# GestaltCogTeam/STEP

Hardware: AMD Instinct MI355X
Metric: training windows/sec on PEMS04, horizon-12 MAE parity, 1/2/4/8 MI355X (higher is better)
Workload: dtype f16 (TSFormer Q/K/weights) + bf16 (P, V, GraphWaveNet / graph-learner GEMMs) operands, f32 accumulate

## Files before the change

include/step_hip.h:

```cpp
#ifndef STEP_HIP_H
#define STEP_HIP_H

#include <stdint.h>

#ifdef __cplusplus
extern "C" {
#endif

const char* step_last_error(void);
int step_abi_version(void);

typedef struct StepGemm {
    int M, N, K, batch;
    const void* A; long sam, sak, sab; int a_bf16;
    const void* B; long sbk, sbn, sbb; int b_bf16;
    float* C; long ldc, scn, scb;
    float alpha;
    int accumulate;
    const float* bias; int relu;
    int splitk;
    int a_kblk; long a_kstride;
    int b_kblk; long b_kstride;
    int b_nblk; long b_nstride;
    int c_nblk; long c_nstride;
// ... 34 lines not shown
    float *fc_w, *fc_b;
    float *bn1_w, *bn1_b, *bn1_rm, *bn1_rv;
    float *bn2_w, *bn2_b, *bn2_rm, *bn2_rv;
    float *bn3_w, *bn3_b, *bn3_rm, *bn3_rv;
    float *fc_out_w, *fc_out_b;
    float *fc_cat_w, *fc_cat_b;
    int gemm_bf16;
} StepDglParams;

long step_dgl_global_saved_floats(int N, int T);
long step_dgl_global_work_floats(int N, int T, int backward);
int step_dgl_global_forward(const float* series_nt, int N, int T, const StepDglParams* p, int training,
                            float momentum, float* saved, float* work, float* g, void* stream);
int step_dgl_global_backward(const float* series_nt, int N, int T, const StepDglParams* p, const float* saved,
                             const float* dg, float* work, const StepDglParams* grads, void* stream);
#define STEP_DGL_FRESH_FC_GRAD 16
int step_dgl_global_backward_phase(const float* series_nt, int N, int T, const StepDglParams* p, const float* saved,
                             const float* dg, float* work, const StepDglParams* grads, int phase, void* stream);

typedef struct StepDglShard { int own1; double count1, count2; } StepDglShard;
int step_dgl_global_forward_shard(const float* series_slice, int N, int Ts, const StepDglParams* p, int training, float momentum,
                                  float* saved, float* work, double* sums, float* g, const StepDglShard* shard, int phase,
                                  void* stream);
int step_dgl_global_backward_shard(const float* series_slice, int N, int Ts, const StepDglParams* p, const float* saved,
                                   const float* dg, float* work, const StepDglParams* grads, const StepDglShard* shard, int phase,
                                   void* stream);
long step_dgl_global_offset(int N, int T, int item);

long step_dgl_edges_saved_floats(int B, int N);
long step_dgl_edges_work_floats(int N);
long step_dgl_edges_theta_offset(int N);
int step_dgl_edges_forward(const float* g, int N, int B, const StepDglParams* p, const float* u, uint64_t seed,
                           float temperature, float* saved, float* theta_out, float* adj_out, void* stream);
int step_dgl_edges_backward(const float* g, int N, int B, const StepDglParams* p, const float* saved,
                            const float* dtheta, const float* dadj, float temperature, float* work,
                            const StepDglParams* grads, float* dg, void* aux_stream, void* stream);

typedef struct StepGwnetParams {
    float *nodevec1, *nodevec2;
    float *start_w, *start_b;
    float *filter_w[8], *filter_b[8];
    float *gate_w[8], *gate_b[8];
    float *skip_w[8], *skip_b[8];
    float *bn_w[8], *bn_b[8], *bn_rm[8], *bn_rv[8];
    float *gconv_w[8], *gconv_b[8];
    float *fc_his0_w, *fc_his0_b, *fc_his2_w, *fc_his2_b;
    float *end1_w, *end1_b, *end2_w, *end2_b;
    int gemm_bf16;
} StepGwnetParams;

long step_gwnet_saved_floats(int B, int N, int dropout);
long step_gwnet_work_floats(int B, int N, int backward);
long step_gwnet_saved_offset(int B, int N, int dropout, int item, int layer);
int step_gwnet_forward(const float* hist, int B, int N, int Cin, const float* hidden_last, const float* adj,
                       const StepGwnetParams* p, int training, float dropout_p, uint64_t seed, float momentum,
                       float* saved, float* work, float* pred, void* stream);
int step_gwnet_forward_phase(const float* hist, int B, int N, int Cin, const float* hidden_last, const float* adj,
                             const StepGwnetParams* p, int training, float dropout_p, uint64_t seed, float momentum,
                             float* saved, float* work, float* pred, int phase, void* stream);
int step_gwnet_backward(const float* hist, int B, int N, int Cin, const float* hidden_last, const StepGwnetParams* p,
                        const float* saved, float* work, const float* dpred, const StepGwnetParams* grads,
                        float* dadj, int dropout, void* aux_stream, void* leaf_stream, void* stream);

int step_pt_dropout(const float* x, float* y, long n, float p, uint64_t seed, uint32_t site, void* stream);
int step_pt_ffn_hidden_fwd(const float* x, const float* w1, const float* b1, long R, float p, uint64_t seed, uint32_t site,
                           uint16_t* hidden, void* stream);
int step_pt_ffn_hidden_bwd(const float* dy, const float* w2, const uint16_t* hidden, long R, float p, uint16_t* dhidden, void* stream);
int step_pt_colsum_bf16(const uint16_t* x, long rows, int cols, float* out, void* stream);
long step_pt_rows_linear_pack_bytes(int nkc, int nog);
int step_pt_rows_linear_pack(const float* w, long swo, long swi, int nkc, int nog, const float* bias, void* pack, void* stream);
int step_pt_rows_linear(const void* x, int x_bf16, long R, const void* pack, int nkc, int nog, void* y, int y_bf16, int accumulate, void* stream);
int step_pt_layer_pack(const float* wi, const float* bi, const float* wo, const float* bo, const float* w1, const float* b1, const float* w2,
                       const float* b2, void* ffn, void* qkv, void* o, void* da, void* dx, void* stream);
long step_pt_proj_wgrad_ws_floats(long R);
int step_pt_proj_wgrad(const float* x, const uint16_t* dqkv, const float* dov, const uint16_t* a, long R, float* ws, float* dwi, float* dbi, float* dwo,
                       void* stream);
int step_pt_ffn_fused_fwd_ln(const float* h1, long R, const void* pack, float p, const uint64_t* pool, long pool_words, uint64_t seed, uint32_t site_hidden,
                             uint32_t site_out, const float* gamma, const float* beta, float* pre, float* y, float* stats, void* stream);
int step_pt_rows_linear_ln(const uint16_t* x, long R, const void* pack, const float* res, float p, uint64_t seed, uint32_t site, const float* gamma,
                           const float* beta, float* pre, float* y, float* stats, void* stream);
int step_pt_embed_unmasked_fwd(const float* series, const int* um, const float* w, const float* b, const float* pos, long S, int L, int Pu, float p,
                               uint64_t seed, uint32_t site, float* x, void* stream);
int step_pt_embed_unmasked_bwd(const float* dx, const float* series, const int* um, long S, int L, int Pu, float p, uint64_t seed, uint32_t site,
                               float* dpos, float* dw, float* db, void* stream);
int step_pt_dec_input_bwd_sums(const float* dout, long S, int P, int Pu, float p, uint64_t seed, uint32_t site, const int* midx, float* dz, float* dpos,
                               float* dmask, void* stream);
long step_pt_ffn_pack_bytes(void);
long step_pt_ffn_wgrad_workgroups(long R);
long step_pt_ffn_wgrad_ws_floats(long R);
int step_pt_ffn_pack(const float* w1, const float* b1, const float* w2, const float* b2, void* pack, void* stream);
int step_pt_ffn_fused_fwd(const float* h1, long R, const void* pack, float p, const uint64_t* pool, long pool_words, uint64_t seed, uint32_t site,
                          float* f2, void* stream);
int step_pt_ffn_fused_bwd_data(const float* df2, const float* h1, long R, const void* pack, float p, const uint64_t* pool, long pool_words,
                               uint64_t seed, uint32_t site, float* dh1, void* stream);
int step_pt_ffn_fused_bwd_weights(const float* df2, const float* h1, long R, const void* pack, const float* b1, float p, const uint64_t* pool,
                                  long pool_words, uint64_t seed, uint32_t site, float* ws, float* dw1, float* db1, float* dw2, void* stream);
int step_pt_dropout_relu_mask(float* d, const float* relu_of, long n, float p, uint64_t seed, uint32_t site, void* stream);
int step_pt_add_dropout(const float* a, const float* b, float* out, long n, float p, uint64_t seed, uint32_t site, void* stream);
int step_pt_add_rows(float* x, long S, int P, const float* vec, const int* idx, void* stream);
int step_pt_sum_over_seq(const float* dx, long S, int ldp, int p_off, int p_cnt, const int* idx, float* dvec, void* stream);
int step_pt_token_gather(const float* src, long S, int P, const int* idx, int T, float scale, float* dst, void* stream);
int step_pt_token_scatter(const float* ddst, long S, int P, const int* idx, int T, float scale, float* dsrc, void* stream);
int step_pt_dec_input(const float* z, const float* mask_token, const float* pos, const int* midx, long S, int P, int Pu,
                      float p, uint64_t seed, uint32_t site, float* out, void* stream);
int step_pt_dec_input_bwd(const float* dout, long S, int P, int Pu, float p, uint64_t seed, uint32_t site, float* dz,
                          float* dm, void* stream);
// ... 97 lines not shown
```

step_amd/_lib.py:

```python
import ctypes
import os

import torch

_HERE = os.path.dirname(os.path.abspath(__file__))
LIB_PATH = os.environ.get("STEP_HIP_LIB") or os.path.join(_HERE, "libstep_hip.so")

_vp, _i, _l, _f, _u64 = ctypes.c_void_p, ctypes.c_int, ctypes.c_long, ctypes.c_float, ctypes.c_uint64


class StepGemm(ctypes.Structure):
    _fields_ = [("M", _i), ("N", _i), ("K", _i), ("batch", _i),
                ("A", _vp), ("sam", _l), ("sak", _l), ("sab", _l), ("a_bf16", _i),
                ("B", _vp), ("sbk", _l), ("sbn", _l), ("sbb", _l), ("b_bf16", _i),
                ("C", _vp), ("ldc", _l), ("scn", _l), ("scb", _l),
                ("alpha", _f), ("accumulate", _i), ("bias", _vp), ("relu", _i), ("splitk", _i),
                ("a_kblk", _i), ("a_kstride", _l), ("b_kblk", _i), ("b_kstride", _l),
                ("b_nblk", _i), ("b_nstride", _l), ("c_nblk", _i), ("c_nstride", _l),
                ("a_kscale", _vp), ("a_kshift", _vp), ("a_kperiod", _i),
                ("batch0", _i), ("sab1", _l), ("sbb1", _l), ("scb1", _l), ("compute_bf16", _i), ("a_rowsum", _vp), ("c_nscale", _vp), ("c_nshift", _vp), ("c_mvec", _vp),
                ("c_nperiod", _i), ("splitk_ws", _vp), ("splitk_ws_floats", _l)]


class StepDglParams(ctypes.Structure):
# ... 7 lines not shown
    _fields_ = [("nodevec1", _vp), ("nodevec2", _vp), ("start_w", _vp), ("start_b", _vp),
                ("filter_w", _vp * 8), ("filter_b", _vp * 8), ("gate_w", _vp * 8), ("gate_b", _vp * 8),
                ("skip_w", _vp * 8), ("skip_b", _vp * 8),
                ("bn_w", _vp * 8), ("bn_b", _vp * 8), ("bn_rm", _vp * 8), ("bn_rv", _vp * 8),
                ("gconv_w", _vp * 8), ("gconv_b", _vp * 8),
                ("fc_his0_w", _vp), ("fc_his0_b", _vp), ("fc_his2_w", _vp), ("fc_his2_b", _vp),
                ("end1_w", _vp), ("end1_b", _vp), ("end2_w", _vp), ("end2_b", _vp), ("gemm_bf16", _i)]


_PD = ctypes.POINTER(StepDglParams)


class StepDynState(ctypes.Structure):
    _fields_ = [("seed_xor", ctypes.c_uint64), ("adam_step", ctypes.c_int32), ("lr", _f), ("gsl_coef", _f), ("reserved", _f)]


class StepDglShard(ctypes.Structure):
    _fields_ = [("own1", ctypes.c_int), ("count1", ctypes.c_double), ("count2", ctypes.c_double)]


_PS = ctypes.POINTER(StepDglShard)
_PG = ctypes.POINTER(StepGwnetParams)

_SIGS = {
    "step_last_error": (ctypes.c_char_p, []),
    "step_abi_version": (_i, []),
    "step_gemm": (_i, [ctypes.POINTER(StepGemm), _vp]),
    "step_tsformer_encode": (_i, [_vp, _i, _i, _vp, _l, _i, _i, _vp, _vp, _vp, _vp, _f, _vp, _l, _u64, _vp, _vp]),
    "step_dropout_pool_fill": (_i, [_vp, _l, _f, _u64, _vp]),
    "step_tsformer_dropout_words": (_l, [_i, _i]),
    "step_gather_windows": (_i, [_vp, _i, _i, _i, _i, _vp, _i, _i, _i, _vp, _vp, _vp, _vp]),
    "step_pack_long_history": (_i, [_vp, _i, _i, _i, _i, _i, _vp, _vp]),
    "step_knn_workspace_bytes": (_l, [_i, _i, _i]),
    "step_knn_graph": (_i, [_vp, _vp, _i, _i, _i, _i, _vp, _vp, _vp, _l, _vp]),
    "step_topk_mask": (_i, [_vp, _i, _i, _i, _vp, _vp, _l, _vp]),
    "step_selftest_mfma": (_i, [_vp, _vp]),
    "step_streams_concurrent": (_i, [_vp, _vp, ctypes.POINTER(_i)]),
    "step_dgl_global_saved_floats": (_l, [_i, _i]),
    "step_dgl_global_work_floats": (_l, [_i, _i, _i]),
    "step_dgl_global_forward": (_i, [_vp, _i, _i, _PD, _i, _f, _vp, _vp, _vp, _vp]),
    "step_dgl_global_backward": (_i, [_vp, _i, _i, _PD, _vp, _vp, _vp, _PD, _vp]),
    "step_dgl_global_backward_phase": (_i, [_vp, _i, _i, _PD, _vp, _vp, _vp, _PD, _i, _vp]),
    "step_dgl_global_forward_shard": (_i, [_vp, _i, _i, _PD, _i, _f, _vp, _vp, _vp, _vp, _PS, _i, _vp]),
    "step_dgl_global_backward_shard": (_i, [_vp, _i, _i, _PD, _vp, _vp, _vp, _PD, _PS, _i, _vp]),
    "step_dgl_global_offset": (_l, [_i, _i, _i]),
    "step_dgl_edges_saved_floats": (_l, [_i, _i]),
    "step_dgl_edges_work_floats": (_l, [_i]),
    "step_dgl_edges_theta_offset": (_l, [_i]),
    "step_dgl_edges_forward": (_i, [_vp, _i, _i, _PD, _vp, _u64, _f, _vp, _vp, _vp, _vp]),
    "step_dgl_edges_backward": (_i, [_vp, _i, _i, _PD, _vp, _vp, _vp, _f, _vp, _PD, _vp, _vp, _vp]),
    "step_gwnet_saved_floats": (_l, [_i, _i, _i]),
    "step_gwnet_work_floats": (_l, [_i, _i, _i]),
    "step_gwnet_saved_offset": (_l, [_i, _i, _i, _i, _i]),
    "step_gwnet_forward": (_i, [_vp, _i, _i, _i, _vp, _vp, _PG, _i, _f, _u64, _f, _vp, _vp, _vp, _vp]),
    "step_gwnet_forward_phase": (_i, [_vp, _i, _i, _i, _vp, _vp, _PG, _i, _f, _u64, _f, _vp, _vp, _vp, _i, _vp]),
    "step_gwnet_backward": (_i, [_vp, _i, _i, _i, _vp, _PG, _vp, _vp, _vp, _PG, _vp, _i, _vp, _vp, _vp]),
    "step_pt_dropout": (_i, [_vp, _vp, _l, _f, _u64, ctypes.c_uint32, _vp]),
    "step_pt_ffn_hidden_fwd": (_i, [_vp, _vp, _vp, _l, _f, _u64, ctypes.c_uint32, _vp, _vp]),
    "step_pt_ffn_hidden_bwd": (_i, [_vp, _vp, _vp, _l, _f, _vp, _vp]),
    "step_pt_colsum_bf16": (_i, [_vp, _l, _i, _vp, _vp]),
    "step_pt_rows_linear_pack_bytes": (_l, [_i, _i]),
    "step_pt_rows_linear_pack": (_i, [_vp, _l, _l, _i, _i, _vp, _vp, _vp]),
    "step_pt_rows_linear": (_i, [_vp, _i, _l, _vp, _i, _i, _vp, _i, _i, _vp]),
    "step_pt_layer_pack": (_i, [_vp] * 14),
    "step_pt_proj_wgrad_ws_floats": (_l, [_l]),
    "step_pt_proj_wgrad": (_i, [_vp, _vp, _vp, _vp, _l, _vp, _vp, _vp, _vp, _vp]),
    "step_pt_ffn_fused_fwd_ln": (_i, [_vp, _l, _vp, _f, _vp, _l, _u64, ctypes.c_uint32, ctypes.c_uint32, _vp, _vp, _vp, _vp, _vp, _vp]),
    "step_pt_rows_linear_ln": (_i, [_vp, _l, _vp, _vp, _f, _u64, ctypes.c_uint32, _vp, _vp, _vp, _vp, _vp, _vp]),
    "step_pt_embed_unmasked_fwd": (_i, [_vp, _vp, _vp, _vp, _vp, _l, _i, _i, _f, _u64, ctypes.c_uint32, _vp, _vp]),
    "step_pt_embed_unmasked_bwd": (_i, [_vp, _vp, _vp, _l, _i, _i, _f, _u64, ctypes.c_uint32, _vp, _vp, _vp, _vp]),
    "step_pt_dec_input_bwd_sums": (_i, [_vp, _l, _i, _i, _f, _u64, ctypes.c_uint32, _vp, _vp, _vp, _vp, _vp]),
    "step_pt_ffn_pack_bytes": (_l, []),
    "step_pt_ffn_wgrad_workgroups": (_l, [_l]),
    "step_pt_ffn_wgrad_ws_floats": (_l, [_l]),
    "step_pt_ffn_pack": (_i, [_vp, _vp, _vp, _vp, _vp, _vp]),
    "step_pt_ffn_fused_fwd": (_i, [_vp, _l, _vp, _f, _vp, _l, _u64, ctypes.c_uint32, _vp, _vp]),
    "step_pt_ffn_fused_bwd_data": (_i, [_vp, _vp, _l, _vp, _f, _vp, _l, _u64, ctypes.c_uint32, _vp, _vp]),
    "step_pt_ffn_fused_bwd_weights": (_i, [_vp, _vp, _l, _vp, _vp, _f, _vp, _l, _u64, ctypes.c_uint32, _vp, _vp, _vp, _vp, _vp]),
    "step_pt_add_layernorm_fwd": (_i, [_vp, _vp, _l, _f, _u64, ctypes.c_uint32, _vp, _vp, _vp, _vp, _vp, _vp]),
    "step_pt_layernorm_bwd_dropout": (_i, [_vp, _vp, _l, _vp, _vp, _vp, _vp, _f, _u64, ctypes.c_uint32, _vp, _vp, _vp, _vp]),
    "step_pt_dropout_relu_mask": (_i, [_vp, _vp, _l, _f, _u64, ctypes.c_uint32, _vp]),
    "step_pt_add_dropout": (_i, [_vp, _vp, _vp, _l, _f, _u64, ctypes.c_uint32, _vp]),
    "step_pt_add_rows": (_i, [_vp, _l, _i, _vp, _vp, _vp]),
    "step_pt_sum_over_seq": (_i, [_vp, _l, _i, _i, _i, _vp, _vp, _vp]),
    "step_pt_token_gather": (_i, [_vp, _l, _i, _vp, _i, _f, _vp, _vp]),
    "step_pt_token_scatter": (_i, [_vp, _l, _i, _vp, _i, _f, _vp, _vp]),
    "step_pt_dec_input": (_i, [_vp, _vp, _vp, _vp, _l, _i, _i, _f, _u64, ctypes.c_uint32, _vp, _vp]),
    "step_pt_dec_input_bwd": (_i, [_vp, _l, _i, _i, _f, _u64, ctypes.c_uint32, _vp, _vp, _vp]),
    "step_pt_layernorm_fwd": (_i, [_vp, _l, _vp, _vp, _vp, _vp, _vp]),
    "step_pt_layernorm_bwd": (_i, [_vp, _vp, _l, _vp, _vp, _vp, _vp, _vp, _vp]),
    "step_pt_attention_fwd": (_i, [_vp, _l, _i, _f, _u64, ctypes.c_uint32, _vp, _vp, _vp]),
    "step_pt_attention_bwd": (_i, [_vp, _vp, _vp, _vp, _l, _i, _f, _u64, ctypes.c_uint32, _vp, _vp]),
    "step_pt_attention_fwd_bf16": (_i, [_vp, _l, _i, _f, _u64, ctypes.c_uint32, _vp, _vp, _vp, _vp, _l, _vp]),
    "step_pt_attention_bwd_bf16": (_i, [_vp, _vp, _vp, _vp, _l, _i, _f, _u64, ctypes.c_uint32, _vp, _vp, _vp]),
    "step_pt_linear_bf16out": (_i, [_vp, _vp, _l, _l, _vp, _l, _i, _i, _vp, _vp]),
    "step_pt_relu_mask": (_i, [_vp, _vp, _l, _vp]),
    "step_colsum": (_i, [_vp, _l, _i, _l, _vp, _vp]),
    "step_loss_fwd_bwd": (_i, [_vp, _vp, _l, _vp, _vp, _l, _f, _f, _vp, _vp, _vp, _vp, _vp]),
    "step_loss_scaled_fwd_bwd": (_i, [_vp, _vp, _l, _l, _f, _f, _vp, _vp, _l, _f, _f, _vp, _vp, _vp, _vp, _vp]),
    "step_scale2": (_i, [_vp, _l, _vp, _l, _vp, _vp, _vp, _vp]),
    "step_masked_metrics": (_i, [_vp, _l, _vp, _l, _l, _f, _vp, _vp, _vp]),
    "step_adam_work_floats": (_l, []),
    "step_adam_clip": (_i, [_vp, _vp, _vp, _vp, _l, _f, _f, _f, _f, _f, _i, _f, _vp, _vp, _vp]),
    "step_adam_clip_sharded": (_i, [_vp, _vp, _vp, _vp, _l, _f, _f, _f, _f, _f, _i, _f, _vp, _vp, _vp, _vp]),
    "step_comm_available": (_i, []),
    "step_comm_version": (_i, []),
# ... 107 lines not shown
```

step_amd/csrc/gwnet.hip:

```cpp
#include "common.h"
#include "step_internal.h"
#include <vector>

namespace {

constexpr int C = 32, CAT = 224, CS = 256, CE = 512, OUT = 12, NL = 8, HID = 96;
constexpr int TIN[NL] = {13, 12, 10, 9, 7, 6, 4, 3};
constexpr int DIL[NL] = {1, 2, 1, 2, 1, 2, 1, 2};
constexpr int TOUT[NL] = {12, 10, 9, 7, 6, 4, 3, 1};

__global__ void start_conv_kernel(const float* __restrict__ hist, int B, int N, int Cin, const float* __restrict__ w,
                                  const float* __restrict__ b, float* __restrict__ x0) {
    long idx = (long)blockIdx.x * 256 + threadIdx.x;
    long total = (long)B * N * 13 * C;
    if (idx >= total) return;
    int c = idx % C, t = (idx / C) % 13;
    long bn = idx / (C * 13);
    int n = bn % N, bb = bn / N;
    float v = b[c];
    if (t >= 1) {
        const float* src = hist + (((long)bb * 12 + (t - 1)) * N + n) * Cin;
        v += w[c * 2] * src[0] + w[c * 2 + 1] * src[1];
    }
    x0[idx] = v;
// ... 529 lines not shown
        for (int e = 0; e < 16; ++e) acc[e] = 0.f;
#pragma unroll
        for (int q = 0; q < 4; ++q) mma16<BF16>(acc, dp[q >> 1][q & 1], b[q]);
#pragma unroll
        for (int e = 0; e < 16; ++e) dxs[(wave & 1) * 32 + (e & 3) + 8 * (e >> 2) + 4 * h][32 * nt + col] = acc[e];
    }
    __syncthreads();
    const int c = threadIdx.x & 31, jg = threadIdx.x >> 5;
    float s1 = 0.f, s2 = 0.f;
    const float mean = statprev ? statprev[64 + c] : 0.f, rstd = statprev ? statprev[96 + c] : 0.f;
    const int njt = G * Tin;
    for (int j0 = 0; j0 < njt; j0 += 32) {
        float dr[4], yv[4], v[4];
        long o[4];
        bool valid[4];
#pragma unroll
        for (int u = 0; u < 4; ++u) {
            const int j = j0 + 8 * u + jg;
            const int g = j / Tin, t = j - g * Tin;
            const long bnr = bn0 + g;
            valid[u] = j < njt && bnr < BN;
            const long bc = valid[u] ? bnr : 0;
            const int tc = valid[u] ? t : 0;
            o[u] = (bc * Tin + tc) * C + c;
            const bool tap1 = valid[u] && tc >= dil;
            dr[u] = (dres && tap1) ? dres[(bc * Tout + tc - dil) * C + c] : 0.f;
            yv[u] = yprev ? yprev[o[u]] : 0.f;
            float x = 0.f;
            if (valid[u] && tc < Tout) x += dxs[g * Tout + tc][c];
            if (tap1) x += dxs[g * Tout + tc - dil][32 + c];
            v[u] = x;
        }
#pragma unroll
        for (int u = 0; u < 4; ++u) {
            if (!valid[u]) continue;
            const float x = v[u] + dr[u];
            dx[o[u]] = x;
            s1 += x; s2 += x * (yv[u] - mean) * rstd;
        }
    }
    if (!yprev) return;
    red[jg][c] = s1; red[jg][32 + c] = s2;
    __syncthreads();
    if (threadIdx.x < 64) {
        float a = 0.f;
#pragma unroll
        for (int r = 0; r < 8; ++r) a += red[r][threadIdx.x];
        bsum[threadIdx.x] = a;
    }
    __syncthreads();
    add_block_sums(sums, bsum);
}

__global__ void im2col_kernel(XIn x, long BN, int Tin, int Tout, int dil, float* __restrict__ xcat) {
    long idx = (long)blockIdx.x * 256 + threadIdx.x;
    if (idx >= BN * Tout * 64) return;
    int k = idx % 64, t = (idx / 64) % Tout;
    long bn = idx / (64L * Tout);
    float v = x.src[(bn * Tin + t + (k >> 5) * dil) * C + (k & 31)];
    if (x.stat) v = v * x.stat[k & 31] + x.stat[32 + (k & 31)];
    xcat[idx] = v;
}
__global__ void unpack_skip_grad_kernel(const float* __restrict__ dwskip, SkipPtrs G) {
    const int o = blockIdx.x, k = threadIdx.x;
    G.w[k >> 5][o * C + (k & 31)] += dwskip[o * CS + k];
}
__global__ void head_combine_kernel(const float* __restrict__ skip, const float* __restrict__ h2, long n, float* __restrict__ xh) {
    long idx = (long)blockIdx.x * 256 + threadIdx.x;
    if (idx >= n) return;
    xh[idx] = fmaxf(skip[idx] + h2[idx], 0.f);
}
struct MPtr8 { float* p[8]; };
__global__ void add_to8_kernel(MPtr8 dst, const float* __restrict__ v, int n) {
    int i = blockIdx.x * 256 + threadIdx.x;
    if (i >= n) return;
    const float x = v[i];
#pragma unroll
    for (int k = 0; k < 8; ++k) dst.p[k][i] += x;
}
__global__ void relu_bwd_kernel(float* __restrict__ d, const float* __restrict__ y, long n) {
    long idx = (long)blockIdx.x * 256 + threadIdx.x;
    if (idx < n && !(y[idx] > 0.f)) d[idx] = 0.f;
}

__global__ __launch_bounds__(256) void rowsum_mod_kernel(const float* __restrict__ x, int cols, int mod, float* __restrict__ out) {
    __shared__ float red[4];
    const long row = blockIdx.x;
    float s = 0.f;
    for (int j = threadIdx.x; j < cols; j += 256) s += x[row * cols + j];
    s = wave_sum(s);
    if ((threadIdx.x & 63) == 0) red[threadIdx.x >> 6] = s;
    __syncthreads();
    if (threadIdx.x == 0) atomicAdd(&out[row % mod], red[0] + red[1] + red[2] + red[3]);
}

constexpr int ADJ_NSEG = 2 * (12 + 10 + 9 + 7 + 6 + 4 + 3);
struct AdjOffsets { long cat[NL - 1], dcat[NL - 1]; };
__global__ void adj_ktab_kernel(AdjOffsets o, int N, GemmKSeg* __restrict__ tab) {
    const int j = threadIdx.x, s = blockIdx.x;
    if (j >= ADJ_NSEG) return;
    constexpr int tout[NL - 1] = {12, 10, 9, 7, 6, 4, 3};
    int i = 0, rem = j >> 1;
    while (rem >= tout[i]) { rem -= tout[i]; ++i; }
    const int t = rem, pair = j & 1, T = tout[i];
    GemmKSeg g;
    g.a_off = o.cat[i] + (long)t * CAT + (pair == 0 ? (1 + 2 * s) * C : 0);
    g.b_off = o.dcat[i] + (long)t * CAT + (pair == 0 ? (2 + 2 * s) * C : (1 + 2 * s) * C);
    g.a_rs = g.b_rs = T * CAT;
    g.a_bs = g.b_bs = (long)N * T * CAT;
    tab[s * ADJ_NSEG + j] = g;
}

inline dim3 g1(long n) { return dim3((unsigned)((n + 255) / 256)); }

// ... 4 lines not shown
    float* take(long n) {
        float* p = base ? base + used : nullptr;
        used += (n + 3) & ~3L;
        return p;
    }
};

static inline int n8(int N) { return (N + 7) & ~7; }
static inline bool hop_transposed_operand(int N) {
    static const int min_n = []() { const char* e = getenv("STEP_HOP_XT_MIN_N"); return e ? atoi(e) : 768; }();
    return N >= min_n;
}

struct Saved {
    float *x0, *cat[NL], *tf[NL], *sg[NL], *y[NL], *mask[NL], *bnstat[NL], *zlast;
    float *Pstk, *PTstk, *Pa, *Madp, *rs, *cs;
    uint16_t *P16, *PT16;
    float *skip, *h1, *h2, *xh, *e1;
    long total;
};
Saved carve_saved(float* base, int B, int N, bool dropout) {
    Carver cv(base);
    Saved s;
    const long BN = (long)B * N;
    s.x0 = cv.take(BN * TIN[0] * C);
    s.zlast = cv.take(BN * CS);
    for (int i = 0; i < NL; ++i) {
        s.cat[i] = cv.take(BN * TOUT[i] * CAT);
        s.tf[i] = cv.take(BN * TOUT[i] * C);
        s.sg[i] = cv.take(BN * TOUT[i] * C);
        s.y[i] = i < NL - 1 ? cv.take(BN * TOUT[i] * C) : nullptr;
        s.mask[i] = (i < NL - 1 && dropout) ? cv.take(BN * TOUT[i] * C) : nullptr;
        s.bnstat[i] = cv.take(128);
    }
    s.Pstk = cv.take(3L * B * N * N);
    s.PTstk = cv.take(3L * B * N * N);
    s.P16 = (uint16_t*)cv.take(3L * B * N * n8(N) / 2);
    s.PT16 = (uint16_t*)cv.take(3L * B * N * n8(N) / 2);
    s.Pa = cv.take((long)N * N);
    s.Madp = cv.take((long)N * N);
    s.rs = cv.take(BN);
    s.cs = cv.take(BN);
    s.skip = cv.take(BN * CS);
    s.h1 = cv.take(BN * CE);
    s.h2 = cv.take(BN * CS);
    s.xh = cv.take(BN * CS);
    s.e1 = cv.take(BN * CE);
    s.total = cv.used;
    return s;
}
struct Work {
    float *wcat, *wcatT, *bcat, *wskip, *wmixT, *dwcat, *dbcat, *dwskip;
    double* acc64;
    float *xcat[NL], *bsum, *y7, *m7;
    uint16_t* xT;
    float *dcat[NL - 1], *dpre[NL], *dh[NL - 1], *dres, *dxa, *dxb, *dskip, *dPstk, *dPa, *dM, *rf, *rb;
    GemmKSeg* ktab;
    float *d_e1, *d_xh, *d_h2, *d_h1;
    long total;
};
Work carve_work(float* base, int B, int N, bool backward) {
    Carver cv(base);
    Work w;
    const long BN = (long)B * N;
    w.wcat = cv.take(NL * 64 * 64);
    w.wcatT = cv.take(NL * 64 * 64);
    w.bcat = cv.take(NL * 64);
    w.wskip = cv.take(CS * CS);
    w.wmixT = cv.take(7 * C * CAT);
    w.dwcat = cv.take(NL * 64 * 64);
    w.dbcat = cv.take(NL * 64);
    w.dwskip = cv.take(CS * CS);
    w.acc64 = (double*)cv.take(2L * NL * NCOPY * 64);
    w.xT = hop_transposed_operand(N) ? (uint16_t*)cv.take(3L * B * 12 * C * n8(N) / 2) : nullptr;
    for (int i = 0; i < NL; ++i) w.xcat[i] = backward ? cv.take(BN * TOUT[i] * 64) : nullptr;
    w.bsum = cv.take(CS);
    w.y7 = cv.take(BN * TOUT[NL - 1] * C);
    w.m7 = cv.take(BN * TOUT[NL - 1] * C);
    if (backward) {
        for (int i = 0; i < NL - 1; ++i) w.dcat[i] = cv.take(BN * TOUT[i] * CAT);
        w.ktab = (GemmKSeg*)cv.take(3L * ADJ_NSEG * sizeof(GemmKSeg) / sizeof(float));
        for (int i = 0; i < NL; ++i) w.dpre[i] = cv.take(BN * TOUT[i] * 64);
        for (int i = 0; i < NL - 1; ++i) w.dh[i] = cv.take(BN * TOUT[i] * C);
        w.dres = cv.take(BN * 12 * C);
        w.dxa = cv.take(BN * 13 * C);
        w.dxb = cv.take(BN * 13 * C);
        w.dskip = cv.take(BN * CS);
        w.dPstk = cv.take(3L * B * N * N);
        w.dPa = cv.take((long)N * N);
        w.dM = cv.take((long)N * N);
        w.rf = cv.take(BN > N ? BN : N);
        w.rb = cv.take(BN);
        w.d_e1 = cv.take(BN * CE);
        w.d_xh = cv.take(BN * CS);
        w.d_h2 = cv.take(BN * CS);
        w.d_h1 = cv.take(BN * CE);
    }
    w.total = cv.used;
    return w;
}

int zero(float* p, long n, hipStream_t st) {
    if (hipMemsetAsync(p, 0, (size_t)n * sizeof(float), st) != hipSuccess) {
        step_set_error("gwnet: memset failed");
        return STEP_ERR_HIP;
    }
    return STEP_OK;
}

int nconv_fwd3(const float* Pstk, const uint16_t* PT16, float* cat, int src0, int sstep, int dst0, int B, int N, int T, int bf16,
               uint16_t* xT, hipStream_t st) {
    StepGemm g = gemm_desc(N, T * C, N, Pstk, 1, N, cat + src0 * C, (long)T * CAT, 1, cat + dst0 * C, (long)T * CAT);
    if (bf16 && xT) {
        const int nsrc = sstep == 0 ? 1 : 3;
        slots_to_bf16T_kernel<<<dim3(cdiv(N, 64), T, nsrc * B), 256, 0, st>>>(cat, src0, sstep, B, N, T, n8(N), xT);
        STEP_LAUNCH_CHECK("slots_to_bf16T");
        g.batch = 3 * B; g.batch0 = B;
        g.A = PT16; g.a_bf16 = 1; g.sam = n8(N); g.sak = 1; g.sab = (long)N * n8(N); g.sab1 = (long)B * N * n8(N);
        g.B = xT; g.b_bf16 = 1; g.sbk = 1; g.sbn = n8(N); g.sbb = (long)T * C * n8(N); g.sbb1 = nsrc == 1 ? 0 : (long)B * T * C * n8(N);
        g.scb = (long)N * T * CAT; g.scb1 = 2L * C;
        g.c_nblk = C; g.c_nstride = CAT;
        g.compute_bf16 = 1;
        return step_gemm_launch(g, st);
    }
    g.batch = 3 * B; g.batch0 = B;
    g.sab = (long)N * N; g.sab1 = (long)B * N * N;
    if (bf16) { g.A = PT16; g.a_bf16 = 1; g.sam = n8(N); g.sak = 1; g.sab = (long)N * n8(N); g.sab1 = (long)B * N * n8(N); }
    g.sbb = (long)N * T * CAT; g.sbb1 = (long)sstep * C;
    g.scb = (long)N * T * CAT; g.scb1 = 2L * C;
    g.b_nblk = C; g.b_nstride = CAT; g.c_nblk = C; g.c_nstride = CAT;
    g.compute_bf16 = bf16;
    return step_gemm_launch(g, st);
}
int nconv_bwd_data3(const float* PTstk, const uint16_t* P16, float* dcat, int src0, int dst0, int dstep, int B, int N, int T, int bf16,
                    uint16_t* xT, hipStream_t st) {
    StepGemm g = gemm_desc(N, T * C, N, PTstk, 1, N, dcat + src0 * C, (long)T * CAT, 1, dcat + dst0 * C, (long)T * CAT);
    if (bf16 && xT) {
        slots_to_bf16T_kernel<<<dim3(cdiv(N, 64), T, 3 * B), 256, 0, st>>>(dcat, src0, 2, B, N, T, n8(N), xT);
        STEP_LAUNCH_CHECK("slots_to_bf16T");
        g.batch = 3 * B; g.batch0 = B;
        g.A = P16; g.a_bf16 = 1; g.sam = n8(N); g.sak = 1; g.sab = (long)N * n8(N); g.sab1 = (long)B * N * n8(N);
        g.B = xT; g.b_bf16 = 1; g.sbk = 1; g.sbn = n8(N); g.sbb = (long)T * C * n8(N); g.sbb1 = (long)B * T * C * n8(N);
        g.scb = (long)N * T * CAT; g.scb1 = (long)dstep * C;
        g.c_nblk = C; g.c_nstride = CAT;
        g.accumulate = dstep == 0 ? 2 : 1;
        g.compute_bf16 = 1;
        return step_gemm_launch(g, st);
    }
    g.batch = 3 * B; g.batch0 = B;
    g.sab = (long)N * N; g.sab1 = (long)B * N * N;
    if (bf16) { g.A = P16; g.a_bf16 = 1; g.sam = n8(N); g.sak = 1; g.sab = (long)N * n8(N); g.sab1 = (long)B * N * n8(N); }
    g.sbb = (long)N * T * CAT; g.sbb1 = 2L * C;
    g.scb = (long)N * T * CAT; g.scb1 = (long)dstep * C;
    g.b_nblk = C; g.b_nstride = CAT; g.c_nblk = C; g.c_nstride = CAT;
    g.accumulate = dstep == 0 ? 2 : 1;
    g.compute_bf16 = bf16;
    return step_gemm_launch(g, st);
}
}

extern "C" long step_gwnet_saved_floats(int B, int N, int dropout) { return carve_saved(nullptr, B, N, dropout != 0).total; }
extern "C" long step_gwnet_work_floats(int B, int N, int backward) { return carve_work(nullptr, B, N, backward != 0).total; }
extern "C" long step_gwnet_saved_offset(int B, int N, int dropout, int item, int layer) {
    Saved s = carve_saved((float*)16, B, N, dropout != 0);
    float* p = item == 0 ? s.mask[layer] : item == 1 ? s.y[layer] : s.bnstat[layer];
    return p ? (long)(p - (float*)16) : -1;
}

template <bool BF16>
static int gwnet_layers_forward(const StepGwnetParams* p, const Saved& S, const Work& W, int B, int N, bool training, float drop_p,
                                uint64_t seed, float momentum, bool dead_bn7, const StepDynState* dyn, hipStream_t st,
                                bool first_tcn_only = false, bool skip_first_tcn = false) {
    const long BN = (long)B * N;
    for (int i = 0; i < (first_tcn_only ? 1 : NL); ++i) {
        const int Tin = TIN[i], Tout = TOUT[i], dil = DIL[i];
        const long npos = BN * Tout;
        BnFwd bn = {nullptr, nullptr, nullptr, nullptr, training ? 1 : 0, momentum, nullptr, (double)BN * Tin, nullptr};
        if (i > 0) {
            bn.gamma = p->bn_w[i - 1]; bn.beta = p->bn_b[i - 1]; bn.rm = p->bn_rm[i - 1]; bn.rv = p->bn_rv[i - 1];
            bn.stat = S.bnstat[i - 1]; bn.sums = W.acc64 + (long)(i - 1) * NCOPY * 64;
        }
        if (!(i == 0 && skip_first_tcn)) {
            tcn_fwd_kernel<BF16><<<(unsigned)cdiv(npos, 128), 256, 0, st>>>(i == 0 ? S.x0 : S.y[i - 1], bn, npos, Tin, Tout, dil, W.wcat + i * 4096,
                                                                            W.bcat + i * 64, S.tf[i], S.sg[i], S.cat[i], S.zlast, i);
            STEP_LAUNCH_CHECK("tcn_fwd");
        }
        if (first_tcn_only) break;
        if (i == NL - 1 && !(dead_bn7 && training)) break;
        STEP_TRY(nconv_fwd3(S.Pstk, S.PT16, S.cat[i], 0, 0, 1, B, N, Tout, BF16, W.xT, st));
        STEP_TRY(nconv_fwd3(S.Pstk, S.PT16, S.cat[i], 1, 2, 2, B, N, Tout, BF16, W.xT, st));
        const XIn xin = {i == 0 ? S.x0 : S.y[i - 1], i == 0 ? nullptr : S.bnstat[i - 1]};
        const bool dead = i == NL - 1;
        mix_fwd_kernel<BF16><<<(unsigned)cdiv(npos, 64), 256, 0, st>>>(S.cat[i], p->gconv_w[i], p->gconv_b[i], xin, npos, Tin, Tout, dil, drop_p,
                                                                       (uint32_t)seed, (uint32_t)(seed >> 32), (uint32_t)i, dead ? W.m7 : S.mask[i],
                                                                       dead ? W.y7 : S.y[i], W.acc64 + (long)i * NCOPY * 64, dyn);
        STEP_LAUNCH_CHECK("mix_fwd");
        if (dead) {
            const BnFwd b7 = {p->bn_w[i], p->bn_b[i], p->bn_rm[i], p->bn_rv[i], 1, momentum, S.bnstat[i], (double)npos, W.acc64 + (long)i * NCOPY * 64};
            bn_stats_only_kernel<<<1, 64, 0, st>>>(b7);
            STEP_LAUNCH_CHECK("bn7_stats");
        }
    }
    return STEP_OK;
}

static int pack_weights(const StepGwnetParams* p, const Work& W, hipStream_t st) {
    GatePtrs gp;
    SkipPtrs sp;
    MixPtrs mp;
    for (int i = 0; i < NL; ++i) {
        gp.wf[i] = p->filter_w[i]; gp.bf[i] = p->filter_b[i]; gp.wg[i] = p->gate_w[i]; gp.bg[i] = p->gate_b[i];
        sp.w[i] = p->skip_w[i]; sp.b[i] = p->skip_b[i];
        if (i < NL - 1) mp.w[i] = p->gconv_w[i];
    }
    pack_weights_kernel<<<384 + 7 * 28, 256, 0, st>>>(gp, sp, mp, W.wcat, W.wcatT, W.bcat, W.wskip, W.bsum, W.wmixT);
// ... 91 lines not shown
        g4.batch = B; g4.sab = (long)N * CE; g4.scb = (long)OUT * N; g4.scn = N;
        g4.bias = p->end2_b;
        g4.compute_bf16 = allbf16; STEP_TRY(step_gemm_launch(g4, st));
    }
    return STEP_OK;
}

template <bool BF16>
static int gwnet_layers_backward(const StepGwnetParams* p, const StepGwnetParams* grads, const Saved& S, const Work& W, int B, int N,
                                 float** dx0, hipStream_t st, AuxLane& lane, AuxLane& leaves, hipEvent_t* adj_done) {
    const long BN = (long)B * N;
    float* dx_next = nullptr;
    float* dxbuf[2] = {W.dxa, W.dxb};
    {
        AdjOffsets o;
        for (int i = 0; i < NL - 1; ++i) { o.cat[i] = S.cat[i] - S.cat[0]; o.dcat[i] = W.dcat[i] - W.dcat[0]; }
        adj_ktab_kernel<<<3, 128, 0, st>>>(o, N, W.ktab);
        STEP_LAUNCH_CHECK("adj_ktab");
    }
    static const bool adj_pieces = []() { const char* e = getenv("STEP_ADJ_PIECES"); return !(e && e[0] == '0'); }();
    bool adj_first = true;
    auto adj_piece = [&](int lo, int hi, hipStream_t on_stream) -> int {
        int seg0 = 0, nseg = 0;
        for (int i = 0; i < lo; ++i) seg0 += 2 * TOUT[i];
        for (int i = lo; i <= hi; ++i) nseg += 2 * TOUT[i];
        StepGemm g = gemm_desc(N, N, 32 * nseg, S.cat[0], 0, 1, W.dcat[0], 1, 0, W.dPstk, N);
        g.batch = 3 * B; g.batch0 = B;
        g.scb = (long)N * N; g.scb1 = (long)B * N * N;
        g.compute_bf16 = BF16;
        g.accumulate = adj_first ? 0 : 1;
        adj_first = false;
        return step_gemm_segmented_launch(g, W.ktab + seg0, ADJ_NSEG, on_stream);
    };
    for (int i = NL - 1; i >= 0; --i) {
        const int Tin = TIN[i], Tout = TOUT[i], dil = DIL[i];
        const long npos = BN * Tout;
        const float* cat = S.cat[i];
        if (i < NL - 1) {
            const BnBwd bn = {p->bn_w[i], S.bnstat[i], grads->bn_w[i], grads->bn_b[i], (double)npos, W.acc64 + (long)i * NCOPY * 64};
            mix_bwd_kernel<BF16><<<(unsigned)cdiv(npos, 128), 256, 0, st>>>(dx_next, S.y[i], bn, S.mask[i], W.wmixT + i * (C * CAT), npos, W.dres, W.dh[i],
                                                                            W.dcat[i]);
            STEP_LAUNCH_CHECK("mix_bwd");
            STEP_TRY(nconv_bwd_data3(S.PTstk, S.P16, W.dcat[i], 2, 1, 2, B, N, Tout, BF16, W.xT, st));
            STEP_TRY(nconv_bwd_data3(S.PTstk, S.P16, W.dcat[i], 1, 0, 0, B, N, Tout, BF16, W.xT, st));
            if (adj_pieces && i == 0) { STEP_TRY(adj_piece(0, 0, lane.fork())); *adj_done = lane.done(); }
        }
        float* dx = dxbuf[i & 1];
        tcn_bwd_kernel<BF16><<<(unsigned)cdiv(BN, TB_ROWS / Tout), 256, 0, st>>>(i < NL - 1 ? W.dcat[i] : nullptr, W.dskip, i, S.tf[i], S.sg[i],
                                                                                W.wcatT + i * 4096, i < NL - 1 ? W.dres : nullptr, BN, Tin, Tout, dil,
                                                                                W.dpre[i], dx, i > 0 ? S.y[i - 1] : nullptr,
                                                                                i > 0 ? S.bnstat[i - 1] : nullptr,
                                                                                i > 0 ? W.acc64 + (long)(i - 1) * NCOPY * 64 : nullptr);
        STEP_LAUNCH_CHECK("tcn_bwd");
        const XIn xin = {i == 0 ? S.x0 : S.y[i - 1], i == 0 ? nullptr : S.bnstat[i - 1]};
        hipEvent_t ev = leaves.on ? leaves.mark() : lane.mark();
        if (adj_pieces && i == 4) STEP_TRY(adj_piece(4, 6, lane.after(ev)));
        if (adj_pieces && i == 2) STEP_TRY(adj_piece(2, 3, lane.after(ev)));
        if (adj_pieces && i == 1) STEP_TRY(adj_piece(1, 1, lane.after(ev)));
        hipStream_t leaf = leaves.after(ev);
        if (i < NL - 1) {
            StepGemm gw = gemm_desc(C, CAT, (int)npos, W.dh[i], 1, C, cat, CAT, 1, grads->gconv_w[i], CAT);
            gw.accumulate = 2; gw.splitk = -1;
            gw.a_rowsum = grads->gconv_b[i];
            gw.compute_bf16 = BF16; STEP_TRY(step_gemm_launch(gw, leaf));
        }
        im2col_kernel<<<g1(npos * 64), 256, 0, leaf>>>(xin, BN, Tin, Tout, dil, W.xcat[i]);
        STEP_LAUNCH_CHECK("im2col");
        StepGemm gw = gemm_desc(64, 64, (int)npos, W.dpre[i], 1, 64, W.xcat[i], 64, 1, W.dwcat + i * 4096, 64);
        gw.accumulate = 2; gw.splitk = -1;
        gw.a_rowsum = W.dbcat + i * 64;
        gw.compute_bf16 = BF16; STEP_TRY(step_gemm_launch(gw, leaf));
        dx_next = dx;
    }
    *dx0 = dx_next;
    if (!adj_pieces) STEP_TRY(adj_piece(0, NL - 2, lane.fork()));
    return STEP_OK;
}

extern "C" int step_gwnet_backward(const float* hist, int B, int N, int Cin, const float* hidden_last, const StepGwnetParams* p,
                                   const float* saved, float* work, const float* dpred, const StepGwnetParams* grads,
                                   float* dadj, int dropout, void* aux_stream, void* leaf_stream, void* stream) {
    STEP_REQUIRE(hist && hidden_last && p && saved && work && dpred && grads && dadj, "gwnet_backward: null argument");
    STEP_REQUIRE(B > 0 && N > 0 && Cin >= 2, "gwnet_backward: bad sizes");
    hipStream_t st = (hipStream_t)stream;
    AuxLane lane(st, (hipStream_t)aux_stream);
    AuxLane leaves(st, leaf_stream ? (hipStream_t)leaf_stream : (hipStream_t)aux_stream, 64);
    Saved S = carve_saved((float*)saved, B, N, dropout != 0);
    Work W = carve_work(work, B, N, true);
    const long BN = (long)B * N;
    const int allbf16 = p->gemm_bf16;
    auto split_for = [](long) { return -1; };

    STEP_TRY(pack_weights(p, W, st));
    STEP_TRY(zero(W.dwcat, (long)((float*)W.acc64 - W.dwcat) + 2L * NL * NCOPY * 64, st));
    const long NN = (long)N * N;

    {
        StepGemm g = gemm_desc(N, CE, OUT, dpred, 1, N, p->end2_w, CE, 1, W.d_e1, CE);
        g.batch = B; g.sab = (long)OUT * N; g.scb = (long)N * CE;
        STEP_TRY(step_gemm_launch(g, st));
        relu_bwd_kernel<<<g1(BN * CE), 256, 0, st>>>(W.d_e1, S.e1, BN * CE);
        StepGemm gx = gemm_desc((int)BN, CS, CE, W.d_e1, CE, 1, p->end1_w, CS, 1, W.d_xh, CS);
        gx.compute_bf16 = allbf16; STEP_TRY(step_gemm_launch(gx, st));
        relu_bwd_kernel<<<g1(BN * CS), 256, 0, st>>>(W.d_xh, S.xh, BN * CS);
        {
            hipStream_t leaf = leaves.fork();
            StepGemm gz = gemm_desc((int)BN, CS, CS, W.d_xh, CS, 1, W.wskip, CS, 1, W.dskip, CS);
            gz.compute_bf16 = allbf16; STEP_TRY(step_gemm_launch(gz, st));
            {
                StepGemm gw = gemm_desc(OUT, CE, N, dpred, N, 1, S.e1, CE, 1, grads->end2_w, CE);
                gw.batch = B; gw.sab = (long)OUT * N; gw.sbb = (long)N * CE; gw.scb = 0; gw.accumulate = 2;
                STEP_TRY(step_gemm_launch(gw, leaf));
                rowsum_mod_kernel<<<B * OUT, 256, 0, leaf>>>(dpred, N, OUT, grads->end2_b);
                STEP_LAUNCH_CHECK("end2_bias_grad");
                StepGemm gw1 = gemm_desc(CE, CS, (int)BN, W.d_e1, 1, CE, S.xh, CS, 1, grads->end1_w, CS);
                gw1.accumulate = 2; gw1.splitk = split_for(BN);
                gw1.a_rowsum = grads->end1_b;
                gw1.compute_bf16 = allbf16; STEP_TRY(step_gemm_launch(gw1, leaf));
            }
            STEP_TRY(zero(W.bsum, CS, leaf));
            STEP_TRY(step_colsum_launch(W.d_xh, BN, CS, CS, W.bsum, leaf));
            MPtr8 gb;
            for (int i = 0; i < NL; ++i) gb.p[i] = grads->skip_b[i];
            add_to8_kernel<<<1, 256, 0, leaf>>>(gb, W.bsum, CS);
            StepGemm gws = gemm_desc(CS, CS, (int)BN, W.d_xh, 1, CS, S.zlast, CS, 1, W.dwskip, CS);
            gws.accumulate = 2; gws.splitk = split_for(BN);
            gws.compute_bf16 = allbf16; STEP_TRY(step_gemm_launch(gws, leaf));
            if (hipMemcpyAsync(W.d_h2, W.d_xh, (size_t)BN * CS * sizeof(float), hipMemcpyDeviceToDevice, leaf) != hipSuccess) {
// ... 59 lines not shown
```

Before: 2334.

## Batch GraphWaveNet weight-gradient GEMMs into two fused multi-layer kernels with implicit im2col

The per-layer weight-gradient work in GraphWaveNet backward used to be an im2col kernel plus a generic GEMM for the dilated conv, and a separate GEMM for the graph-conv mixing weights, each launched per layer on a leaf stream. That is replaced by two kernels issued once after the layer loop: one covering all TCN layers, which builds the im2col operand on the fly and applies BN scale/shift, and one covering all mix layers. Both use MFMA tiles, reduce through LDS and commit with global atomics. This removes the xcat scratch buffers and many small launches, and moves the adjacency pieces to plain forks. In exchange, weight-gradient work no longer overlaps with the per-layer backward, and the atomic float accumulation order becomes nondeterministic.

New measurement: 2326. No clear change (-0.3%).

```diff
diff --git a/include/step_hip.h b/include/step_hip.h
--- a/include/step_hip.h
+++ b/include/step_hip.h
@@ -110,6 +110,7 @@
 long step_gwnet_saved_floats(int B, int N, int dropout);
 long step_gwnet_work_floats(int B, int N, int backward);
 long step_gwnet_saved_offset(int B, int N, int dropout, int item, int layer);
+int step_gwnet_wgrad_positions(void);
 int step_gwnet_forward(const float* hist, int B, int N, int Cin, const float* hidden_last, const float* adj,
                        const StepGwnetParams* p, int training, float dropout_p, uint64_t seed, float momentum,
                        float* saved, float* work, float* pred, void* stream);
diff --git a/step_amd/_lib.py b/step_amd/_lib.py
--- a/step_amd/_lib.py
+++ b/step_amd/_lib.py
@@ -83,6 +83,7 @@
     "step_gwnet_saved_floats": (_l, [_i, _i, _i]),
     "step_gwnet_work_floats": (_l, [_i, _i, _i]),
     "step_gwnet_saved_offset": (_l, [_i, _i, _i, _i, _i]),
+    "step_gwnet_wgrad_positions": (_i, []),
     "step_gwnet_forward": (_i, [_vp, _i, _i, _i, _vp, _vp, _PG, _i, _f, _u64, _f, _vp, _vp, _vp, _vp]),
     "step_gwnet_forward_phase": (_i, [_vp, _i, _i, _i, _vp, _vp, _PG, _i, _f, _u64, _f, _vp, _vp, _vp, _i, _vp]),
     "step_gwnet_backward": (_i, [_vp, _i, _i, _i, _vp, _PG, _vp, _vp, _vp, _PG, _vp, _i, _vp, _vp, _vp]),
diff --git a/step_amd/csrc/gwnet.hip b/step_amd/csrc/gwnet.hip
--- a/step_amd/csrc/gwnet.hip
+++ b/step_amd/csrc/gwnet.hip
@@ -605,14 +605,127 @@
     add_block_sums(sums, bsum);
 }
 
-__global__ void im2col_kernel(XIn x, long BN, int Tin, int Tout, int dil, float* __restrict__ xcat) {
-    long idx = (long)blockIdx.x * 256 + threadIdx.x;
-    if (idx >= BN * Tout * 64) return;
-    int k = idx % 64, t = (idx / 64) % Tout;
-    long bn = idx / (64L * Tout);
-    float v = x.src[(bn * Tin + t + (k >> 5) * dil) * C + (k & 31)];
-    if (x.stat) v = v * x.stat[k & 31] + x.stat[32 + (k & 31)];
-    xcat[idx] = v;
+constexpr int WG_POS = 512;
+__device__ __forceinline__ float wgrad_operand(float v, bool bf16) { return bf16 ? bf16_bits_to_f32(f32_to_bf16_bits(v)) : v; }
+__device__ __forceinline__ void wgrad_tile_to_lds(float* red, int ld, int r0, int c0, const f32x16& acc, int col, int h) {
+#pragma unroll
+    for (int e = 0; e < 16; ++e) atomicAdd(&red[(r0 + (e & 3) + 8 * (e >> 2) + 4 * h) * ld + c0 + col], acc[e]);
+}
+
+struct TcnWgradArgs {
+    const float *dpre[NL], *x[NL], *stat[NL];
+    long npos[NL];
+    int wg_end[NL], tin[NL], tout[NL], dil[NL];
+};
+template <bool BF16>
+__global__ __launch_bounds__(256) void tcn_wgrad_kernel(TcnWgradArgs A, float* __restrict__ dwcat, float* __restrict__ dbcat) {
+    __shared__ float red[64 * 64 + 64];
+    int L = 0;
+    while (L < NL - 1 && (int)blockIdx.x >= A.wg_end[L]) ++L;
+    const long p_beg = (long)((int)blockIdx.x - (L ? A.wg_end[L - 1] : 0)) * WG_POS;
+    const long p_end = min(A.npos[L], p_beg + WG_POS);
+    const int Tin = A.tin[L], Tout = A.tout[L], dil = A.dil[L];
+    const float *dpre = A.dpre[L], *x = A.x[L], *stat = A.stat[L];
+    for (int i = threadIdx.x; i < 64 * 64 + 64; i += 256) red[i] = 0.f;
+    __syncthreads();
+    const int lane = threadIdx.x & 63, wave = threadIdx.x >> 6, col = lane & 31, h = lane >> 5;
+    const float sc = stat ? stat[col] : 1.f, sh = stat ? stat[32 + col] : 0.f;
+    f32x16 acc[2][2];
+#pragma unroll
+    for (int e = 0; e < 16; ++e) { acc[0][0][e] = 0.f; acc[0][1][e] = 0.f; acc[1][0][e] = 0.f; acc[1][1][e] = 0.f; }
+    float bs[2] = {0.f, 0.f};
+    for (long pb = p_beg + 16 * wave; pb < p_end; pb += 64) {
+        const long p0 = pb + 8 * h;
+        const long pc = min(p0, p_end - 1);
+        long bn = pc / Tout;
+        int t = (int)(pc - bn * Tout);
+        float a[2][8], b[2][8];
+#pragma unroll
+        for (int j = 0; j < 8; ++j) {
+            const long p = bn * Tout + t, xrow = bn * Tin + t;
+            a[0][j] = dpre[p * 64 + col]; a[1][j] = dpre[p * 64 + 32 + col];
+            b[0][j] = x[xrow * C + col]; b[1][j] = x[(xrow + dil) * C + col];
+            if (p0 + j + 1 < p_end && ++t == Tout) { t = 0; ++bn; }
+        }
+#pragma unroll
+        for (int j = 0; j < 8; ++j) {
+            const bool ok = p0 + j < p_end;
+            if (stat) { b[0][j] = b[0][j] * sc + sh; b[1][j] = b[1][j] * sc + sh; }
+            a[0][j] = ok ? a[0][j] : 0.f; a[1][j] = ok ? a[1][j] : 0.f;
+            b[0][j] = ok ? b[0][j] : 0.f; b[1][j] = ok ? b[1][j] : 0.f;
+            bs[0] += wgrad_operand(a[0][j], BF16); bs[1] += wgrad_operand(a[1][j], BF16);
+        }
+#pragma unroll
+        for (int qo = 0; qo < 2; ++qo)
+#pragma unroll
+            for (int tap = 0; tap < 2; ++tap) mma16<BF16>(acc[qo][tap], a[qo], b[tap]);
+    }
+    if (p_beg + 16 * wave < p_end) {
+#pragma unroll
+        for (int qo = 0; qo < 2; ++qo) {
+#pragma unroll
+            for (int tap = 0; tap < 2; ++tap) wgrad_tile_to_lds(red, 64, 32 * qo, 32 * tap, acc[qo][tap], col, h);
+            const float s = bs[qo] + __shfl_xor(bs[qo], 32, 64);
+            if (h == 0) atomicAdd(&red[64 * 64 + 32 * qo + col], s);
+        }
+    }
+    __syncthreads();
+    for (int i = threadIdx.x; i < 64 * 64; i += 256) unsafeAtomicAdd(dwcat + L * 4096 + i, red[i]);
+    if (threadIdx.x < 64) unsafeAtomicAdd(dbcat + L * 64 + threadIdx.x, red[64 * 64 + threadIdx.x]);
+}
+
+struct MixWgradArgs {
+    const float *dh[NL - 1], *cat[NL - 1];
+    float *dw[NL - 1], *db[NL - 1];
+    long npos[NL - 1];
+    int wg_end[NL - 1];
+};
+template <bool BF16>
+__global__ __launch_bounds__(256) void mix_wgrad_kernel(MixWgradArgs A) {
+    __shared__ float red[C * CAT + C];
+    int L = 0;
+    while (L < NL - 2 && (int)blockIdx.x >= A.wg_end[L]) ++L;
+    const long p_beg = (long)((int)blockIdx.x - (L ? A.wg_end[L - 1] : 0)) * WG_POS;
+    const long p_end = min(A.npos[L], p_beg + WG_POS);
+    const float *dh = A.dh[L], *cat = A.cat[L];
+    for (int i = threadIdx.x; i < C * CAT + C; i += 256) red[i] = 0.f;
+    __syncthreads();
+    const int lane = threadIdx.x & 63, wave = threadIdx.x >> 6, col = lane & 31, h = lane >> 5;
+    f32x16 acc[7];
+#pragma unroll
+    for (int s = 0; s < 7; ++s)
+#pragma unroll
+        for (int e = 0; e < 16; ++e) acc[s][e] = 0.f;
+    float bs = 0.f;
+    for (long pb = p_beg + 16 * wave; pb < p_end; pb += 64) {
+        const long p0 = pb + 8 * h;
+        float a[8], b[7][8];
+#pragma unroll
+        for (int j = 0; j < 8; ++j) {
+            const bool ok = p0 + j < p_end;
+            const long p = ok ? p0 + j : p_end - 1;
+            const float av = dh[p * C + col];
+            a[j] = ok ? av : 0.f;
+            bs += wgrad_operand(a[j], BF16);
+#pragma unroll
+            for (int s = 0; s < 7; ++s) {
+                const float bv = cat[p * CAT + 32 * s + col];
+                b[s][j] = ok ? bv : 0.f;
+            }
+        }
+#pragma unroll
+        for (int s = 0; s < 7; ++s) mma16<BF16>(acc[s], a, b[s]);
+    }
+    if (p_beg + 16 * wave < p_end) {
+#pragma unroll
+        for (int s = 0; s < 7; ++s) wgrad_tile_to_lds(red, CAT, 0, 32 * s, acc[s], col, h);
+        const float s = bs + __shfl_xor(bs, 32, 64);
+        if (h == 0) atomicAdd(&red[C * CAT + col], s);
+    }
+    __syncthreads();
+    float *dw = A.dw[L], *db = A.db[L];
+    for (int i = threadIdx.x; i < C * CAT; i += 256) unsafeAtomicAdd(dw + i, red[i]);
+    if (threadIdx.x < C) unsafeAtomicAdd(db + threadIdx.x, red[C * CAT + threadIdx.x]);
 }
 __global__ void unpack_skip_grad_kernel(const float* __restrict__ dwskip, SkipPtrs G) {
     const int o = blockIdx.x, k = threadIdx.x;
@@ -723,7 +836,7 @@
 struct Work {
     float *wcat, *wcatT, *bcat, *wskip, *wmixT, *dwcat, *dbcat, *dwskip;
     double* acc64;
-    float *xcat[NL], *bsum, *y7, *m7;
+    float *bsum, *y7, *m7;
     uint16_t* xT;
     float *dcat[NL - 1], *dpre[NL], *dh[NL - 1], *dres, *dxa, *dxb, *dskip, *dPstk, *dPa, *dM, *rf, *rb;
     GemmKSeg* ktab;
@@ -744,7 +857,6 @@
     w.dwskip = cv.take(CS * CS);
     w.acc64 = (double*)cv.take(2L * NL * NCOPY * 64);
     w.xT = hop_transposed_operand(N) ? (uint16_t*)cv.take(3L * B * 12 * C * n8(N) / 2) : nullptr;
-    for (int i = 0; i < NL; ++i) w.xcat[i] = backward ? cv.take(BN * TOUT[i] * 64) : nullptr;
     w.bsum = cv.take(CS);
     w.y7 = cv.take(BN * TOUT[NL - 1] * C);
     w.m7 = cv.take(BN * TOUT[NL - 1] * C);
@@ -832,6 +944,7 @@
 
 extern "C" long step_gwnet_saved_floats(int B, int N, int dropout) { return carve_saved(nullptr, B, N, dropout != 0).total; }
 extern "C" long step_gwnet_work_floats(int B, int N, int backward) { return carve_work(nullptr, B, N, backward != 0).total; }
+extern "C" int step_gwnet_wgrad_positions(void) { return WG_POS; }
 extern "C" long step_gwnet_saved_offset(int B, int N, int dropout, int item, int layer) {
     Saved s = carve_saved((float*)16, B, N, dropout != 0);
     float* p = item == 0 ? s.mask[layer] : item == 1 ? s.y[layer] : s.bnstat[layer];
@@ -1029,28 +1142,33 @@
                                                                                 i > 0 ? S.bnstat[i - 1] : nullptr,
                                                                                 i > 0 ? W.acc64 + (long)(i - 1) * NCOPY * 64 : nullptr);
         STEP_LAUNCH_CHECK("tcn_bwd");
-        const XIn xin = {i == 0 ? S.x0 : S.y[i - 1], i == 0 ? nullptr : S.bnstat[i - 1]};
-        hipEvent_t ev = leaves.on ? leaves.mark() : lane.mark();
-        if (adj_pieces && i == 4) STEP_TRY(adj_piece(4, 6, lane.after(ev)));
-        if (adj_pieces && i == 2) STEP_TRY(adj_piece(2, 3, lane.after(ev)));
-        if (adj_pieces && i == 1) STEP_TRY(adj_piece(1, 1, lane.after(ev)));
-        hipStream_t leaf = leaves.after(ev);
-        if (i < NL - 1) {
-            StepGemm gw = gemm_desc(C, CAT, (int)npos, W.dh[i], 1, C, cat, CAT, 1, grads->gconv_w[i], CAT);
-            gw.accumulate = 2; gw.splitk = -1;
-            gw.a_rowsum = grads->gconv_b[i];
-            gw.compute_bf16 = BF16; STEP_TRY(step_gemm_launch(gw, leaf));
-        }
-        im2col_kernel<<<g1(npos * 64), 256, 0, leaf>>>(xin, BN, Tin, Tout, dil, W.xcat[i]);
-        STEP_LAUNCH_CHECK("im2col");
-        StepGemm gw = gemm_desc(64, 64, (int)npos, W.dpre[i], 1, 64, W.xcat[i], 64, 1, W.dwcat + i * 4096, 64);
-        gw.accumulate = 2; gw.splitk = -1;
-        gw.a_rowsum = W.dbcat + i * 64;
-        gw.compute_bf16 = BF16; STEP_TRY(step_gemm_launch(gw, leaf));
+        if (adj_pieces && i == 4) STEP_TRY(adj_piece(4, 6, lane.fork()));
+        if (adj_pieces && i == 2) STEP_TRY(adj_piece(2, 3, lane.fork()));
+        if (adj_pieces && i == 1) STEP_TRY(adj_piece(1, 1, lane.fork()));
         dx_next = dx;
     }
     *dx0 = dx_next;
     if (!adj_pieces) STEP_TRY(adj_piece(0, NL - 2, lane.fork()));
+    {
+        hipStream_t leaf = leaves.fork();
+        TcnWgradArgs ta;
+        MixWgradArgs ma;
+        int twg = 0, mwg = 0;
+        for (int i = 0; i < NL; ++i) {
+            const long npos = BN * TOUT[i];
+            ta.dpre[i] = W.dpre[i]; ta.x[i] = i == 0 ? S.x0 : S.y[i - 1]; ta.stat[i] = i == 0 ? nullptr : S.bnstat[i - 1];
+            ta.npos[i] = npos; ta.tin[i] = TIN[i]; ta.tout[i] = TOUT[i]; ta.dil[i] = DIL[i];
+            ta.wg_end[i] = twg += cdiv(npos, WG_POS);
+            if (i == NL - 1) break;
+            ma.dh[i] = W.dh[i]; ma.cat[i] = S.cat[i]; ma.dw[i] = grads->gconv_w[i]; ma.db[i] = grads->gconv_b[i];
+            ma.npos[i] = npos;
+            ma.wg_end[i] = mwg += cdiv(npos, WG_POS);
+        }
+        tcn_wgrad_kernel<BF16><<<twg, 256, 0, leaf>>>(ta, W.dwcat, W.dbcat);
+        STEP_LAUNCH_CHECK("tcn_wgrad");
+        mix_wgrad_kernel<BF16><<<mwg, 256, 0, leaf>>>(ma);
+        STEP_LAUNCH_CHECK("mix_wgrad");
+    }
     return STEP_OK;
 }
 
```
